# h33p/ofps

Measured on AMD Instinct MI355X. Metric: Mvectors/s, 1080p 16x16 blocks +-16 full-search SAD, higher is better.
Workload: dtype u8

## Files before the change

### ofps_amd/csrc/common.hpp

```cpp
#pragma once

#include <hip/hip_runtime.h>

#include <cstdarg>
#include <cstddef>
#include <cstdint>
#include <cstdio>
#include <cstring>
#include <string>

#include "../../include/ofps_hip.h"

namespace ofps {

int set_error(ofps_hip_ctx* ctx, int code, const char* fmt, ...);

inline int ticket_id(long number) { return (int)(number & 0x7FFFFFFF); }
inline long ticket_number(long next, int n, int id) {
    for (long k = next - 1; k >= 0 && k >= next - n; --k) if (ticket_id(k) == id) return k;
    return -1;
}

template <class Ticket, int N>
struct TicketRing {
// ... 72 lines not shown
        void* pinned = nullptr;
        int have_vectors = 0, run_detector = 0, run_estimator = 0;
        int gated = 0;
        size_t n_vectors = 0;
        IslandsTicket isl;
    };
    hipEvent_t gate_done = nullptr;
    TicketRing<Ticket, kTickets> ring;
    void release() {
        for (auto& t : ring.entry) { free_host(t.pinned); destroy(t.done); t.isl.release(); }
        for (int k = 0; k < kSlots; ++k) { destroy(uploaded[k]); destroy(slot_read[k]); }
        destroy(copy_stream); destroy(aux_stream); destroy(fork); destroy(join); destroy(gate_done);
    }
    hipError_t sync_side_streams() {
        const hipError_t e = copy_stream ? hipStreamSynchronize(copy_stream) : hipSuccess;
        return e == hipSuccess && aux_stream ? hipStreamSynchronize(aux_stream) : e;
    }
};

struct BatchStream {
    static constexpr int kTickets = 2;
    int w = 0, h = 0;
    void* last_frame = nullptr;
    struct KltPred { bool valid = false; int half = 0, w = 0, h = 0, cell = 0; uint64_t gen = 0; } klt_pred;
    struct Ticket {
        bool pending = false;
        hipEvent_t done = nullptr, uploaded = nullptr, prev_copied = nullptr;
        bool prev_copied_valid = false;
        void* pinned = nullptr; size_t pinned_cap = 0;
        int n = 0, first_has_prev = 0, run_detector = 0, run_estimator = 0;
        int filtered = 0;
        size_t n_vectors = 0;
        IslandsTicket isl;
    };
    TicketRing<Ticket, kTickets> ring;
    void release() { for (auto& t : ring.entry) { free_host(t.pinned); destroy(t.done); destroy(t.uploaded); destroy(t.prev_copied); t.isl.release(); } }
};

struct DenseStream {
    static constexpr int kSlots = 3, kTickets = 2;
    int w = 0, h = 0;
    int fw = 0, fh = 0, fmt = 0;
    long frames = 0;
    uint64_t frames_gen = 0;
    bool fb_params_valid = false; int fb_levels = 0, fb_radius = 0;
    uint64_t frame_serial = 0;
    uint64_t slot_id[kSlots] = {0, 0, 0};
    struct KltPred { bool valid = false; long pair = 0; int fw = 0, fh = 0, cell = 0; unsigned flags = 0; uint64_t gen = 0; } klt_pred;
    hipStream_t copy_stream = nullptr;
    struct Ticket {
        bool pending = false;
        hipEvent_t done = nullptr, uploaded = nullptr;
        void* pinned = nullptr; size_t pinned_cap = 0;
        int have_vectors = 0, gw = 0, gh = 0;
        size_t max_records = 0;
        int fused = 0, run_detector = 0, run_estimator = 0, dim = 0;
        size_t tail_off = 0;
        IslandsTicket isl;
    };
    TicketRing<Ticket, kTickets> ring;
    void* decode_pinned = nullptr; size_t decode_pinned_cap = 0;
    void release() {
        free_host(decode_pinned);
        for (auto& t : ring.entry) { free_host(t.pinned); destroy(t.done); destroy(t.uploaded); t.isl.release(); }
        destroy(copy_stream);
    }
    hipError_t sync_side_streams() { return copy_stream ? hipStreamSynchronize(copy_stream) : hipSuccess; }
};

}

struct ofps_hip_ctx {
    int device = 0;
    hipStream_t own_stream = nullptr;
    hipStream_t stream = nullptr;
    hipEvent_t ev_start = nullptr, ev_stop = nullptr;
    int num_cus = 0;
    int stream_cus = 0;
    int sad_mode = OFPS_HIP_SAD_EXHAUSTIVE;
    char err[512] = {0};

    struct Options {
        int sad_force_block = 0;
        int densify_no_small = 0;
        int almeida_path = 0;
        int almeida_ept = 0;
        int almeida_block = 0;
        int almeida_hier = 1;
        int almeida_fast = -1;
        int almeida_one_xcd = 1;
        int almeida_prof = 0;
        int lk_prof = 0;
        int fb_prepare_ahead = 1;
        int lk_serial = 0;
        int sad_motion_scale = 1;
        int detect_compensate = 0;
        int sad_gate = 0;
        int sad_consistency = 0;
        int sad_levels = 1;
        int sad_predictors = 0;
        int sad_median = 0;
        int sad_intra = 0;
        int sad_cut = 0;
        int sad_split = 0;
        int sad_batch_filter = 0;
        int sad_prefilter = 0;
        int detect_islands = 0;
        int klt_cell = 16, klt_score_radius = 2, klt_min_score = 1, klt_min_eig = 1, klt_max_residual = 0;
        int klt_mean_removal = 0;
        int klt_fb = 0;
        int klt_prediction = 0;
        int klt_batch_prediction = 0;
        int batch_decoder = 0, klt_levels = 4, klt_radius = 7, klt_iters = 10;
        int multi_rccl = 0;
        int test_almeida_fault = 0;
        int test_lk_fall = -1;
        int test_lk_wait_budget = 0;
        int test_lk_order = 0;
    } opt;

    ofps::PipeStream pipe;
    ofps::BatchStream batch;
    ofps::DenseStream dense;
    ofps::FarnebackState fb;
    struct IslandsLast { char* data = nullptr; size_t cap = 0; int K = 0, items = 0, dim = 0; } isl_last;
    uint32_t lk_epoch = 0;
    uint64_t lk_flags_gen = 0;

    uint32_t gran_tag_base = 0;
    uint64_t gran_zeroed_gen = 0;

    struct Scratch { void* p = nullptr; size_t cap = 0; uint64_t gen = 0; };
    static constexpr int kNumScratch = 62;
    Scratch scratch[kNumScratch];
};

namespace ofps {

enum ScratchSlot {
    S_FRAMES = 0, S_ENTRIES, S_BEST, S_FIELD, S_CELLS, S_WORK0, S_WORK1, S_WORK2, S_WORK3, S_RESULT,
    S_QUAT, S_WORK4, S_PIPE_FRAMES, S_PIPE_ENTRIES, S_PIPE_OUT, S_MASK, S_ENTRIES2, S_GRAN, S_SAD_LIST,
    S_ALM_PART, S_ALM_STATE, S_ALM_HYP, S_ALM_COUNTS, S_ALM_SEL, S_ALM_SELN, S_ALM_PROF, S_ALM_RECOVER,
    S_LK_FRAMES, S_BATCH_FRAMES, S_BATCH_ENTRIES, S_BATCH_OUT, S_BATCH_FIELD,
    S_LK_FLAGS,
    S_FB_WORK,
    S_FB_FLOW,
    S_XMAJOR,
    S_LK_MASKS,
    S_SAD_QBEST,
    S_FE_RAW,
    S_FE_RAW_PAIR,
    S_DENSE_REC,
    S_GATE_RAW,
    S_GATE_BEST,
    S_GATE_FLAGS,
    S_COMP,
    S_CONS_FWD,
    S_CONS_BWD,
    S_CONS_BWD_ENT,
    S_HIER_PYR,
    S_HIER_BEST,
    S_HIER_ENT,
    S_SAD_PREF,
    S_MED_KEEP,
    S_INTRA,
    S_ISL_WORK,
// ... 221 lines not shown
```

### ofps_amd/csrc/ctx.hip

```cpp
#include "common.hpp"

#include <cstdlib>

static thread_local char g_init_err[512] = {0};

namespace ofps {

int set_error(ofps_hip_ctx* ctx, int code, const char* fmt, ...) {
    char* dst = ctx ? ctx->err : g_init_err;
    va_list ap;
    va_start(ap, fmt);
    vsnprintf(dst, 512, fmt, ap);
    va_end(ap);
    return code;
}

int check_hip(ofps_hip_ctx* ctx, hipError_t e, const char* what) {
    if (e == hipSuccess) return OFPS_HIP_OK;
    int code = (e == hipErrorOutOfMemory) ? OFPS_HIP_ENOMEM : OFPS_HIP_EDEVICE;
    return set_error(ctx, code, "%s failed: %s", what, hipGetErrorString(e));
}

void* scratch(ofps_hip_ctx* ctx, int slot, size_t bytes) {
    auto& s = ctx->scratch[slot];
    if (bytes == 0) bytes = 16;
    if (s.cap >= bytes) return s.p;
    if (s.p) {
        if (hipStreamSynchronize(ctx->stream) != hipSuccess) {  }
        (void)hipFree(s.p);
        s.p = nullptr; s.cap = 0;
    }
    size_t cap = (bytes + 4095) & ~size_t(4095);
    hipError_t e = hipMalloc(&s.p, cap);
    if (e != hipSuccess) {
        check_hip(ctx, e, "hipMalloc(scratch)");
        s.p = nullptr;
        return nullptr;
    }
    s.cap = cap;
    s.gen += 1;
    return s.p;
}

int apply_option(ofps_hip_ctx* ctx, const char* name, const char* value, bool from_env) {
    auto& o = ctx->opt;
    const ofps_hip_ctx::Options dflt{};
    const bool unset = !value || !*value;
    const int iv = unset ? 0 : atoi(value);
    if (!strcmp(name, "OFPS_HIP_SAD_KERNEL")) {
        if (!unset && strcmp(value, "block") && strcmp(value, "strip"))
            return set_error(ctx, OFPS_HIP_EINVAL, "%s: '%s' is not block|strip", name, value);
        o.sad_force_block = !unset && !strcmp(value, "block");
    } else if (!strcmp(name, "OFPS_HIP_DENSIFY_NO_SMALL")) {
        o.densify_no_small = unset ? dflt.densify_no_small : (iv != 0);
    } else if (!strcmp(name, "OFPS_HIP_ALMEIDA_PATH")) {
        if (unset) o.almeida_path = 0;
        else if (!strcmp(value, "step")) o.almeida_path = 1;
        else if (!strcmp(value, "wg")) o.almeida_path = 2;
        else if (!strcmp(value, "cluster")) o.almeida_path = 3;
        else return set_error(ctx, OFPS_HIP_EINVAL, "%s: '%s' is not step|wg|cluster", name, value);
    } else if (!strcmp(name, "OFPS_HIP_ALMEIDA_EPT")) {
        if (!unset && iv != 1 && iv != 2 && iv != 4 && iv != 8) return set_error(ctx, OFPS_HIP_EINVAL, "%s: %d is not 1|2|4|8", name, iv);
        o.almeida_ept = unset ? 0 : iv;
    } else if (!strcmp(name, "OFPS_HIP_ALMEIDA_BLOCK")) {
        if (!unset && iv != 256 && iv != 1024) return set_error(ctx, OFPS_HIP_EINVAL, "%s: %d is not 256|1024", name, iv);
        o.almeida_block = unset ? 0 : iv;
    } else if (!strcmp(name, "OFPS_HIP_ALMEIDA_HIER")) {
        if (!unset && (iv < 0 || iv > 2)) return set_error(ctx, OFPS_HIP_EINVAL, "%s: %d is not 0|1|2", name, iv);
        o.almeida_hier = unset ? dflt.almeida_hier : iv;
    } else if (!strcmp(name, "OFPS_HIP_ALMEIDA_FAST")) {
        o.almeida_fast = unset ? -1 : (iv != 0);
    } else if (!strcmp(name, "OFPS_HIP_ALMEIDA_ONE_XCD")) {
        o.almeida_one_xcd = unset ? dflt.almeida_one_xcd : (iv != 0);
    } else if (!strcmp(name, "OFPS_HIP_ALMEIDA_PROF")) {
        o.almeida_prof = unset ? 0 : (iv != 0);
    } else if (!strcmp(name, "OFPS_HIP_LK_PROF")) {
        o.lk_prof = unset ? 0 : (iv != 0);
    } else if (!strcmp(name, "OFPS_HIP_FB_PREPARE_AHEAD")) {
        o.fb_prepare_ahead = unset ? dflt.fb_prepare_ahead : (iv != 0);
    } else if (!strcmp(name, "OFPS_HIP_LK_SERIAL")) {
        o.lk_serial = unset ? 0 : (iv != 0);
    } else if (!strcmp(name, "OFPS_HIP_SAD_MOTION_SCALE")) {
        if (!unset && iv != 1 && iv != 4) return set_error(ctx, OFPS_HIP_EINVAL, "%s: %d is not 1|4", name, iv);
        o.sad_motion_scale = unset ? dflt.sad_motion_scale : iv;
    } else if (!strcmp(name, "OFPS_HIP_DETECT_COMPENSATE")) {
        if (!unset && iv != 0 && iv != 1) return set_error(ctx, OFPS_HIP_EINVAL, "%s: %d is not 0|1", name, iv);
        o.detect_compensate = unset ? dflt.detect_compensate : iv;
    } else if (!strcmp(name, "OFPS_HIP_DETECT_ISLANDS")) {
        if (!unset && (iv < 0 || iv > kMaxIslands)) return set_error(ctx, OFPS_HIP_EINVAL, "%s: %d outside [0, %d]", name, iv, kMaxIslands);
        o.detect_islands = unset ? dflt.detect_islands : iv;
    } else if (!strcmp(name, "OFPS_HIP_SAD_GATE")) {
        if (!unset && iv < 0) return set_error(ctx, OFPS_HIP_EINVAL, "%s: %d is negative", name, iv);
        o.sad_gate = unset ? dflt.sad_gate : iv;
    } else if (!strcmp(name, "OFPS_HIP_SAD_CONSISTENCY")) {
        if (!unset && (iv < 0 || iv > kSadConsistencyMax)) return set_error(ctx, OFPS_HIP_EINVAL, "%s: %d outside [0, %d]", name, iv, kSadConsistencyMax);
        o.sad_consistency = unset ? dflt.sad_consistency : iv;
    } else if (!strcmp(name, "OFPS_HIP_SAD_MEDIAN")) {
        if (!unset && (iv < 0 || iv > kSadMedianMax)) return set_error(ctx, OFPS_HIP_EINVAL, "%s: %d outside [0, %d]", name, iv, kSadMedianMax);
        o.sad_median = unset ? dflt.sad_median : iv;
    } else if (!strcmp(name, "OFPS_HIP_SAD_INTRA")) {
        if (!unset && (iv < 0 || iv > kSadIntraMax)) return set_error(ctx, OFPS_HIP_EINVAL, "%s: %d outside [0, %d]", name, iv, kSadIntraMax);
        o.sad_intra = unset ? dflt.sad_intra : iv;
    } else if (!strcmp(name, "OFPS_HIP_SAD_CUT")) {
        if (!unset && (iv < 0 || iv > kSadCutMax)) return set_error(ctx, OFPS_HIP_EINVAL, "%s: %d outside [0, %d]", name, iv, kSadCutMax);
        o.sad_cut = unset ? dflt.sad_cut : iv;
    } else if (!strcmp(name, "OFPS_HIP_SAD_SPLIT")) {
        if (!unset && (iv < 0 || iv > kSadSplitMax)) return set_error(ctx, OFPS_HIP_EINVAL, "%s: %d outside [0, %d]", name, iv, kSadSplitMax);
        o.sad_split = unset ? dflt.sad_split : iv;
    } else if (!strcmp(name, "OFPS_HIP_SAD_LEVELS")) {
        if (!unset && (iv < 1 || iv > 3)) return set_error(ctx, OFPS_HIP_EINVAL, "%s: '%s' is not 1|2|3", name, value);
        o.sad_levels = unset ? dflt.sad_levels : iv;
    } else if (!strcmp(name, "OFPS_HIP_SAD_PREDICTORS")) {
        if (!unset && strcmp(value, "0") && strcmp(value, "1")) return set_error(ctx, OFPS_HIP_EINVAL, "%s: '%s' is not 0|1", name, value);
        o.sad_predictors = unset ? dflt.sad_predictors : iv;
    } else if (!strcmp(name, "OFPS_HIP_SAD_PREFILTER")) {
        if (!unset && (iv < 0 || iv > kSadPrefilterMax)) return set_error(ctx, OFPS_HIP_EINVAL, "%s: %d outside [0, %d]", name, iv, kSadPrefilterMax);
        o.sad_prefilter = unset ? dflt.sad_prefilter : iv;
    } else if (!strcmp(name, "OFPS_HIP_SAD_BATCH_FILTER")) {
        if (!unset && strcmp(value, "0") && strcmp(value, "1")) return set_error(ctx, OFPS_HIP_EINVAL, "%s: '%s' is not 0|1", name, value);
        o.sad_batch_filter = unset ? dflt.sad_batch_filter : iv;
    } else if (!strcmp(name, "OFPS_HIP_BATCH_DECODER")) {
        if (!unset && strcmp(value, "0") && strcmp(value, "1")) return set_error(ctx, OFPS_HIP_EINVAL, "%s: '%s' is not 0|1", name, value);
        o.batch_decoder = unset ? dflt.batch_decoder : iv;
    } else if (!strcmp(name, "OFPS_HIP_KLT_LEVELS")) {
        if (!unset && (iv < 1 || iv > kKltMaxLevels)) return set_error(ctx, OFPS_HIP_EINVAL, "%s: %d outside [1, %d]", name, iv, kKltMaxLevels);
        o.klt_levels = unset ? dflt.klt_levels : iv;
    } else if (!strcmp(name, "OFPS_HIP_KLT_RADIUS")) {
        if (!unset && (iv < 1 || iv > kKltMaxRadius)) return set_error(ctx, OFPS_HIP_EINVAL, "%s: %d outside [1, %d]", name, iv, kKltMaxRadius);
        o.klt_radius = unset ? dflt.klt_radius : iv;
    } else if (!strcmp(name, "OFPS_HIP_KLT_ITERS")) {
        if (!unset && (iv < 1 || iv > kKltMaxIters)) return set_error(ctx, OFPS_HIP_EINVAL, "%s: %d outside [1, %d]", name, iv, kKltMaxIters);
        o.klt_iters = unset ? dflt.klt_iters : iv;
    } else if (!strcmp(name, "OFPS_HIP_KLT_CELL")) {
        if (!unset && iv != 8 && iv != 16 && iv != 32) return set_error(ctx, OFPS_HIP_EINVAL, "%s: %d is not 8|16|32", name, iv);
        o.klt_cell = unset ? dflt.klt_cell : iv;
    } else if (!strcmp(name, "OFPS_HIP_KLT_SCORE_RADIUS")) {
        if (!unset && (iv < 1 || iv > kKltMaxScoreRadius)) return set_error(ctx, OFPS_HIP_EINVAL, "%s: %d outside [1, %d]", name, iv, kKltMaxScoreRadius);
        o.klt_score_radius = unset ? dflt.klt_score_radius : iv;
    } else if (!strcmp(name, "OFPS_HIP_KLT_MIN_SCORE")) {
        if (!unset && iv < 1) return set_error(ctx, OFPS_HIP_EINVAL, "%s: %d is below 1", name, iv);
        o.klt_min_score = unset ? dflt.klt_min_score : iv;
    } else if (!strcmp(name, "OFPS_HIP_KLT_MIN_EIG")) {
        if (!unset && (iv < 1 || iv > kKltMaxMinEig)) return set_error(ctx, OFPS_HIP_EINVAL, "%s: %d outside [1, %d]", name, iv, kKltMaxMinEig);
        o.klt_min_eig = unset ? dflt.klt_min_eig : iv;
    } else if (!strcmp(name, "OFPS_HIP_KLT_MAX_RESIDUAL")) {
        if (!unset && (iv < 0 || iv > kKltMaxResidual)) return set_error(ctx, OFPS_HIP_EINVAL, "%s: %d outside [0, %d]", name, iv, kKltMaxResidual);
        o.klt_max_residual = unset ? dflt.klt_max_residual : iv;
    } else if (!strcmp(name, "OFPS_HIP_KLT_MEAN_REMOVAL")) {
        if (!unset && strcmp(value, "0") && strcmp(value, "1")) return set_error(ctx, OFPS_HIP_EINVAL, "%s: '%s' is not 0|1", name, value);
        o.klt_mean_removal = unset ? dflt.klt_mean_removal : iv;
    } else if (!strcmp(name, "OFPS_HIP_KLT_FB")) {
        if (!unset && (strspn(value, "0123456789") != strlen(value) || strlen(value) > 4 || iv > kKltMaxFb)) return set_error(ctx, OFPS_HIP_EINVAL, "%s: '%s' outside [0, %d]", name, value, kKltMaxFb);
        o.klt_fb = unset ? dflt.klt_fb : iv;
    } else if (!strcmp(name, "OFPS_HIP_KLT_PREDICTION")) {
        if (!unset && strcmp(value, "0") && strcmp(value, "1")) return set_error(ctx, OFPS_HIP_EINVAL, "%s: '%s' is not 0|1", name, value);
        o.klt_prediction = unset ? dflt.klt_prediction : iv;
    } else if (!strcmp(name, "OFPS_HIP_KLT_BATCH_PREDICTION")) {
        if (!unset && strcmp(value, "0") && strcmp(value, "1")) return set_error(ctx, OFPS_HIP_EINVAL, "%s: '%s' is not 0|1", name, value);
        o.klt_batch_prediction = unset ? dflt.klt_batch_prediction : iv;
    } else if (!strcmp(name, "OFPS_HIP_MULTI_RCCL")) {
        o.multi_rccl = unset ? 0 : (iv != 0);
    } else if (!strcmp(name, "OFPS_HIP_ALMEIDA_TEST_FAULT") || !strcmp(name, "OFPS_HIP_LK_TEST_FALL") ||
               !strcmp(name, "OFPS_HIP_LK_TEST_WAIT_BUDGET") || !strcmp(name, "OFPS_HIP_LK_TEST_ORDER")) {
#ifdef OFPS_HIP_TEST_HOOKS
        if (from_env) return OFPS_HIP_OK;
        if (!strcmp(name, "OFPS_HIP_ALMEIDA_TEST_FAULT")) o.test_almeida_fault = unset ? 0 : iv;
        else if (!strcmp(name, "OFPS_HIP_LK_TEST_WAIT_BUDGET")) o.test_lk_wait_budget = unset || iv < 0 ? 0 : iv;
        else if (!strcmp(name, "OFPS_HIP_LK_TEST_ORDER")) o.test_lk_order = unset || iv < 0 || iv > 2 ? 0 : iv;
        else o.test_lk_fall = unset ? -1 : iv;
#else
        if (from_env) return OFPS_HIP_OK;
        return set_error(ctx, OFPS_HIP_EUNSUPPORTED, "%s is a test hook: this library was built without OFPS_HIP_TEST_HOOKS", name);
#endif
    } else {
        return set_error(ctx, OFPS_HIP_EINVAL, "unknown option '%s'", name);
    }
    return OFPS_HIP_OK;
}

static const char* const kOptionNames[] = {
    "OFPS_HIP_SAD_KERNEL", "OFPS_HIP_DENSIFY_NO_SMALL", "OFPS_HIP_ALMEIDA_PATH", "OFPS_HIP_ALMEIDA_EPT", "OFPS_HIP_ALMEIDA_BLOCK",
    "OFPS_HIP_ALMEIDA_HIER", "OFPS_HIP_ALMEIDA_FAST", "OFPS_HIP_ALMEIDA_ONE_XCD", "OFPS_HIP_ALMEIDA_PROF", "OFPS_HIP_LK_PROF", "OFPS_HIP_LK_SERIAL", "OFPS_HIP_FB_PREPARE_AHEAD", "OFPS_HIP_MULTI_RCCL",
    "OFPS_HIP_SAD_MOTION_SCALE", "OFPS_HIP_DETECT_COMPENSATE", "OFPS_HIP_SAD_GATE", "OFPS_HIP_SAD_CONSISTENCY", "OFPS_HIP_SAD_LEVELS",
    "OFPS_HIP_SAD_PREDICTORS", "OFPS_HIP_SAD_PREFILTER", "OFPS_HIP_SAD_MEDIAN", "OFPS_HIP_SAD_BATCH_FILTER",
    "OFPS_HIP_SAD_INTRA", "OFPS_HIP_SAD_CUT", "OFPS_HIP_DETECT_ISLANDS", "OFPS_HIP_SAD_SPLIT",
    "OFPS_HIP_KLT_CELL", "OFPS_HIP_KLT_SCORE_RADIUS", "OFPS_HIP_KLT_MIN_SCORE", "OFPS_HIP_KLT_MIN_EIG", "OFPS_HIP_KLT_MAX_RESIDUAL",
    "OFPS_HIP_BATCH_DECODER", "OFPS_HIP_KLT_LEVELS", "OFPS_HIP_KLT_RADIUS", "OFPS_HIP_KLT_ITERS", "OFPS_HIP_KLT_MEAN_REMOVAL",
    "OFPS_HIP_KLT_FB", "OFPS_HIP_KLT_PREDICTION", "OFPS_HIP_KLT_BATCH_PREDICTION"};

}

extern "C" {

int ofps_hip_api_version(void) { return OFPS_HIP_API_VERSION; }

int ofps_hip_device_count(void) {
    int n = 0;
    if (hipGetDeviceCount(&n) != hipSuccess) return 0;
    return n;
}

static int stream_cu_count(ofps_hip_ctx* ctx, hipStream_t s);

int ofps_hip_init(int device, ofps_hip_ctx** out) {
    if (!out) return ofps::set_error(nullptr, OFPS_HIP_EINVAL, "ofps_hip_init: out is NULL");
    *out = nullptr;
    int n = 0;
    hipError_t e = hipGetDeviceCount(&n);
    if (e != hipSuccess || n <= 0)
        return ofps::set_error(nullptr, OFPS_HIP_EDEVICE,
                               "ofps_hip_init: no HIP device (%s); this backend has no CPU fallback",
                               e == hipSuccess ? "count == 0" : hipGetErrorString(e));
    if (device < 0 || device >= n)
        return ofps::set_error(nullptr, OFPS_HIP_EINVAL, "ofps_hip_init: device %d out of range [0,%d)", device, n);
    hipDeviceProp_t prop;
    e = hipGetDeviceProperties(&prop, device);
    if (e != hipSuccess) return ofps::check_hip(nullptr, e, "hipGetDeviceProperties");
    if (strncmp(prop.gcnArchName, "gfx950", 6) != 0)
        return ofps::set_error(nullptr, OFPS_HIP_EUNSUPPORTED,
                               "ofps_hip_init: device %d is %s; this library ships gfx950 code only", device,
                               prop.gcnArchName);
    auto* ctx = new ofps_hip_ctx();
    ctx->device = device;
    ctx->num_cus = prop.multiProcessorCount;
    if ((e = hipSetDevice(device)) != hipSuccess ||
        (e = hipStreamCreateWithFlags(&ctx->own_stream, hipStreamNonBlocking)) != hipSuccess ||
        (e = hipEventCreate(&ctx->ev_start)) != hipSuccess || (e = hipEventCreate(&ctx->ev_stop)) != hipSuccess) {
        int rc = ofps::check_hip(nullptr, e, "context setup");
        delete ctx;
        return rc;
    }
    ctx->stream = ctx->own_stream;
    ctx->stream_cus = stream_cu_count(ctx, ctx->stream);
    for (const char* name : ofps::kOptionNames)
        if (const char* v = getenv(name)) {
            if (ofps::apply_option(ctx, name, v, true) != OFPS_HIP_OK) {
                fprintf(stderr, "[ofps_hip] warning: ignoring environment variable %s=%s (%s)\n", name, v, ctx->err);
                ctx->err[0] = '\0';
            }
        }
    ofps::cluster_gate_context_created(device);
    *out = ctx;
    return OFPS_HIP_OK;
}

int ofps_hip_set_option(ofps_hip_ctx* ctx, const char* name, const char* value) {
    if (!ctx) return OFPS_HIP_EINVAL;
    OFPS_REQUIRE(ctx, name, "set_option: null name");
    return ofps::apply_option(ctx, name, value, false);
}

int ofps_hip_has_test_hooks(void) {
#ifdef OFPS_HIP_TEST_HOOKS
    return 1;
#else
    return 0;
#endif
}

int ofps_hip_almeida_recoveries(ofps_hip_ctx* ctx, uint64_t* count) {
    if (!ctx || !count) return OFPS_HIP_EINVAL;
    *count = 0;
    const void* d = ctx->scratch[ofps::S_ALM_RECOVER].p;
    if (!d) return OFPS_HIP_OK;
// ... 125 lines not shown
```

### ofps_amd/csrc/sad.hip

```cpp
#include "common.hpp"

#include <cstdlib>
#include <utility>

namespace {

constexpr int kWavesPerWG = 4;

constexpr int pick_stride(int min_s, int k, int ng) {
    for (int s = min_s; s < min_s + 64; ++s)
        if ((k * s) % 32 == ng % 32) return s;
    return min_s | 1;
}

template <int B, int R, int K>
struct SadCfg {
    static_assert(B % 4 == 0 && R % 4 == 0, "tile origin must stay dword aligned");
    static_assert(B * B * 255 <= 65535, "packed u16 SAD accumulators would overflow");
    static constexpr int NCAND = 2 * R + 1;
    static constexpr int NG = (NCAND + 3) / 4;
    static constexpr int NC = (NCAND + K - 1) / K;
    static constexpr int T = NG * NC;
    static constexpr int PASSES = (T + 63) / 64;
    static constexpr int BW = B / 4;
// ... 790 lines not shown
    }
    const int dy0i = blk_on ? (int)((pbest >> 8) & 0xFF) : R, dx0i = blk_on ? (int)(pbest & 0xFF) : R;
    auto key64 = [&](uint32_t sad, int dyi, int dxi) {
        const int dy = dyi - R, dx = dxi - R;
        return ((unsigned long long)((sad << 16) | (uint32_t)(dx * dx + dy * dy)) << 32) | (unsigned long long)(uint32_t)((dyi << 8) | dxi);
    };
    uint32_t U = pde_two_rows(tile, curl, b, dy0i, dx0i, g);
#pragma unroll
    for (int m = 1; m < C::NG; m <<= 1) U += __shfl_xor(U, m, 64);
    if (g == 0) bestk[b] = blk_on ? key64(U, dy0i, dx0i) : ~0ull;
    int nlist = 0;
    {
        int uj[4];
#pragma unroll
        for (int j = 0; j < 4; ++j) uj[j] = colv[j] ? (int)U : -1;
        const unsigned long long below = (1ull << lane) - 1ull;
        typedef unsigned short us2 __attribute__((ext_vector_type(2)));
        const uint32_t u1 = min(U + 1u, 0xFFFFu) * 0x10001u;
        auto any_le = [&](uint32_t v) {
            const us2 m = __builtin_elementwise_min(__builtin_bit_cast(us2, v), __builtin_bit_cast(us2, u1));
            return __builtin_bit_cast(uint32_t, m) ^ u1;
        };
#pragma unroll
        for (int i = 0; i < C::NCAND; ++i) {
            const int dy = -R + i;
            if (y0 + dy >= 0 && y0 + dy + B <= p.H) {
                const uint32_t lo = (uint32_t)acc[i], hi = (uint32_t)(acc[i] >> 32);
                if (!__ballot((any_le(lo) | any_le(hi)) != 0u)) continue;
                const int s4[4] = {(int)(lo & 0xFFFFu), (int)(lo >> 16), (int)(hi & 0xFFFFu), (int)(hi >> 16)};
#pragma unroll
                for (int j = 0; j < 4; ++j) {
                    const bool hit = s4[j] <= uj[j];
                    const unsigned long long mask = __ballot(hit);
                    if (mask) {
                        const int pos = nlist + __popcll(mask & below);
                        if (hit && pos < P::CAP) list[pos] = ((uint32_t)b << 16) | ((uint32_t)i << 8) | (uint32_t)(4 * g + j);
                        nlist += __popcll(mask);
                    }
                }
            }
        }
#pragma unroll
        for (int i = 0; i < C::KE; ++i) {
            const int dyi = g * C::KE + i, dy = dyi - R;
            const bool hit = xok && dy <= R && y0 + dy >= 0 && y0 + dy + B <= p.H && eacc[i] <= U;
            const unsigned long long mask = __ballot(hit);
            if (mask) {
                const int pos = nlist + __popcll(mask & below);
                if (hit && pos < P::CAP) list[pos] = ((uint32_t)b << 16) | ((uint32_t)dyi << 8) | (uint32_t)(2 * R);
                nlist += __popcll(mask);
            }
        }
    }
    __builtin_amdgcn_fence(__ATOMIC_RELEASE, "wavefront");
    __builtin_amdgcn_wave_barrier();
    __builtin_amdgcn_fence(__ATOMIC_ACQUIRE, "wavefront");
    const int n = nlist;
    if (n > P::CAP) {
        if (lane == 0) {
            const uint32_t pos = atomicAdd(&strip_list[0], 1u);
            strip_list[1 + pos] = (uint32_t)strip;
        }
        return;
    }
    constexpr int PER_STEP = 2 * (64 / C::NG);
    for (int base = 0; base < n; base += PER_STEP) {
        const int idx0 = base + lane / C::NG, idx1 = idx0 + 64 / C::NG;
        const uint32_t e0 = list[min(idx0, n - 1)], e1 = list[min(idx1, n - 1)];
        const int bb0 = (int)(e0 >> 16), dyi0 = (int)((e0 >> 8) & 0xFF), dxi0 = (int)(e0 & 0xFF);
        const int bb1 = (int)(e1 >> 16), dyi1 = (int)((e1 >> 8) & 0xFF), dxi1 = (int)(e1 & 0xFF);
        uint32_t s0 = pde_two_rows(tile, curl, bb0, dyi0, dxi0, g);
        uint32_t s1 = pde_two_rows(tile, curl, bb1, dyi1, dxi1, g);
#pragma unroll
        for (int m = 1; m < C::NG; m <<= 1) { s0 += __shfl_xor(s0, m, 64); s1 += __shfl_xor(s1, m, 64); }
        if (g == 0 && idx0 < n) atomicMin(&bestk[bb0], key64(s0, dyi0, dxi0));
        if (g == 0 && idx1 < n) atomicMin(&bestk[bb1], key64(s1, dyi1, dxi1));
    }
    __builtin_amdgcn_fence(__ATOMIC_RELEASE, "wavefront");
    __builtin_amdgcn_wave_barrier();
    __builtin_amdgcn_fence(__ATOMIC_ACQUIRE, "wavefront");
    if (blk_on && g == 0) write_block_result(p, pair, bx, by, B, R, bestk[b]);
}

__global__ __launch_bounds__(64) void sad_generic_kernel(const SadParams p, int B, int R) {
    const int pair = blockIdx.z, by = blockIdx.y, bx = blockIdx.x;
    const uint8_t* __restrict__ prev = p.prev_base + (size_t)pair * p.prev_pitch;
    const uint8_t* __restrict__ cur = p.cur_base + (size_t)pair * p.cur_pitch;
    const int x0 = bx * B, y0 = by * B, n = 2 * R + 1;
    unsigned long long best = ~0ull;
    for (int cand = threadIdx.x; cand < n * n; cand += 64) {
        const int dy = cand / n - R, dx = cand % n - R;
        if (x0 + dx < 0 || x0 + dx + B > p.W || y0 + dy < 0 || y0 + dy + B > p.H) continue;
        uint32_t sad = 0;
        for (int y = 0; y < B; ++y) {
            const uint8_t* cr = cur + (size_t)(y0 + y) * p.stride + x0;
            const uint8_t* pr = prev + (size_t)(y0 + dy + y) * p.stride + x0 + dx;
            for (int x = 0; x < B; ++x) {
                const int d = (int)cr[x] - (int)pr[x];
                sad += (uint32_t)(d < 0 ? -d : d);
            }
        }
        const unsigned long long key = ((unsigned long long)sad << 32) | ((unsigned long long)(dx * dx + dy * dy) << 16) |
                                       (unsigned long long)(((dy + R) << 8) | (dx + R));
        best = key < best ? key : best;
    }
#pragma unroll
    for (int m = 32; m >= 1; m >>= 1) {
        const unsigned long long o = shfl_xor_u64(best, m);
        best = o < best ? o : best;
    }
    if (threadIdx.x == 0) {
        const int sad = (int)(best >> 32);
        const int dy = (int)((best >> 8) & 0xFF) - R, dx = (int)(best & 0xFF) - R;
        const size_t k = ((size_t)pair * p.nby + by) * p.nbx + bx;
        float4 e;
        e.x = (float)(x0 + B / 2 + dx) * p.nx;
        e.y = (float)(y0 + B / 2 + dy) * p.ny;
        e.z = ((float)dx / 1.0f) * (-p.nx);
        e.w = ((float)dy / 1.0f) * (-p.ny);
        p.out_entries[k] = e;
        if (p.out_best) {
            p.out_best[3 * k + 0] = dx;
            p.out_best[3 * k + 1] = dy;
            p.out_best[3 * k + 2] = sad;
        }
    }
}

template <int B, int R, int K>
void launch_qsad(const SadParams& p, int pairs, hipStream_t s) {
    dim3 grid((p.nbx + kWavesPerWG - 1) / kWavesPerWG, p.nby, pairs);
    hipLaunchKernelGGL((sad_qsad_kernel<B, R, K>), grid, dim3(256), 0, s, p);
}

inline void strip_div_magic(SadParams& q, int strips_per_row) {
    q.div_spp = div_magic48((unsigned)strips_per_row * (unsigned)q.nby);
    q.div_spr = div_magic48((unsigned)strips_per_row);
}

template <int B, int R>
void launch_strip(const SadParams& p, int pairs, hipStream_t s) {
    using C = StripCfg<B, R>;
    const int strips_per_row = (p.nbx + C::NB - 1) / C::NB;
    const int total = strips_per_row * p.nby * pairs;
    const int nwg = ((total + kStripWaves - 1) / kStripWaves + 7) / 8 * 8;
    SadParams q = p;
    strip_div_magic(q, strips_per_row);
    hipLaunchKernelGGL((sad_strip_kernel<B, R>), dim3(nwg), dim3(64 * kStripWaves), 0, s, q, strips_per_row, total);
}

int launch_pde_16_16(ofps_hip_ctx* ctx, const SadParams& p, int pairs, hipStream_t s) {
    using C = StripCfg<16, 16>;
    const int strips_per_row = (p.nbx + C::NB - 1) / C::NB;
    const int total = strips_per_row * p.nby * pairs;
    auto* strip_list = static_cast<uint32_t*>(ofps::scratch(ctx, ofps::S_SAD_LIST, (size_t)(total + 1) * sizeof(uint32_t)));
    if (!strip_list) return OFPS_HIP_ENOMEM;
    OFPS_HIP_TRY(ctx, hipMemsetAsync(strip_list, 0, sizeof(uint32_t), s));
    const int nwg = ((total + kStripWaves - 1) / kStripWaves + 7) / 8 * 8;
    hipLaunchKernelGGL(sad_pde_kernel, dim3(nwg), dim3(64 * kStripWaves), 0, s, p, strips_per_row, total, strip_list);
    const int nwg_ind = nwg < 8 * ctx->num_cus ? nwg : 8 * ctx->num_cus;
    SadParams q = p;
    strip_div_magic(q, strips_per_row);
    hipLaunchKernelGGL((sad_strip_list_kernel<16, 16>), dim3(nwg_ind), dim3(64 * kStripWaves), 0, s, q, strips_per_row,
                       (const uint32_t*)strip_list);
    return OFPS_HIP_OK;
}

}

extern "C" {

size_t ofps_hip_sad_block_count(int W, int H, int block) {
    if (W <= 0 || H <= 0 || block <= 0) return 0;
    return (size_t)(W / block) * (size_t)(H / block);
}

}

namespace {
int sad_check_args(ofps_hip_ctx* ctx, const ofps::SadFrames& f, int block, int range) {
    OFPS_REQUIRE(ctx, f.W > 0 && f.H > 0 && f.stride >= f.W, "sad_flow: bad geometry W=%d H=%d stride=%d", f.W, f.H, f.stride);
    OFPS_REQUIRE(ctx, f.stride % 4 == 0 && ((uintptr_t)f.prev_base % 4) == 0 && ((uintptr_t)f.cur_base % 4) == 0 &&
                          f.prev_pitch % 4 == 0 && f.cur_pitch % 4 == 0,
                 "sad_flow: rows must be 4-byte aligned (stride=%d)", f.stride);
    OFPS_REQUIRE(ctx, block >= 1 && block <= 64 && range >= 0 && range <= 64,
                 "sad_flow: block=%d range=%d outside [1,64]/[0,64]", block, range);
    return OFPS_HIP_OK;
}

SadParams sad_params(const ofps::SadFrames& f, int block, void* d_out_entries, void* d_out_best) {
    SadParams p{};
    p.prev_base = f.prev_base; p.cur_base = f.cur_base;
    p.prev_pitch = f.prev_pitch; p.cur_pitch = f.cur_pitch;
    p.W = f.W; p.H = f.H; p.stride = f.stride;
    p.nbx = f.W / block; p.nby = f.H / block;
    p.nx = 1.0f / (float)f.W; p.ny = 1.0f / (float)f.H;
    p.out_entries = static_cast<float4*>(d_out_entries);
    p.out_best = static_cast<int*>(d_out_best);
    return p;
}

int sad_launch(ofps_hip_ctx* ctx, const ofps::SadFrames& f, int pairs, int block, int range, void* d_out_entries, void* d_out_best) {
    const SadParams p = sad_params(f, block, d_out_entries, d_out_best);
    hipStream_t s = ctx->stream;
    const int key = block * 1000 + range;
    const bool force_block = ctx->opt.sad_force_block != 0;
    const bool strip_ok = !force_block && f.stride % 16 == 0 && ((uintptr_t)f.prev_base % 16) == 0 &&
                          ((uintptr_t)f.cur_base % 16) == 0 && f.prev_pitch % 16 == 0 && f.cur_pitch % 16 == 0 &&
                          (long long)p.nbx * p.nby * pairs < (1ll << 28) && (long long)p.nbx * p.nby < (1ll << 20);
    switch (key) {
        case 16016:
            if (strip_ok && ctx->sad_mode == OFPS_HIP_SAD_PRUNED) {
                const int rc = launch_pde_16_16(ctx, p, pairs, s);
                if (rc != OFPS_HIP_OK) return rc;
            } else if (strip_ok) launch_strip<16, 16>(p, pairs, s);
            else launch_qsad<16, 16, 5>(p, pairs, s);
            break;
        case 16008:
            if (strip_ok) launch_strip<16, 8>(p, pairs, s); else launch_qsad<16, 8, 3>(p, pairs, s);
            break;
        case 16032:
            if (strip_ok) launch_strip<16, 32>(p, pairs, s); else launch_qsad<16, 32, 5>(p, pairs, s);
            break;
        case 8032:
            if (strip_ok) launch_strip<8, 32>(p, pairs, s); else launch_qsad<8, 32, 5>(p, pairs, s);
            break;
        case 8016:
            if (strip_ok) launch_strip<8, 16>(p, pairs, s); else launch_qsad<8, 16, 5>(p, pairs, s);
            break;
        case 8008:
            if (strip_ok) launch_strip<8, 8>(p, pairs, s); else launch_qsad<8, 8, 3>(p, pairs, s);
            break;
#define OFPS_STRIP_CASE(BB, RR)                                         \
        case BB * 1000 + RR:                                            \
            if (strip_ok) { launch_strip<BB, RR>(p, pairs, s); break; } \
            [[fallthrough]];
        OFPS_STRIP_CASE(16, 12) OFPS_STRIP_CASE(16, 20) OFPS_STRIP_CASE(16, 24) OFPS_STRIP_CASE(16, 28)
// ... 128 lines not shown
```

Baseline: 525.6.

## Replace two-kernel PDE SAD with single-pass row-chunk pruning kernel

Adds a single kernel for the 16x16 +-16 full search. It computes a partial SAD over a row subset, takes an upper bound from the best candidate's full SAD, and then finishes only the dy chunks that still hold a live candidate, falling back to all chunks once enough rows survive. This replaces the previous PDE kernel plus indirect strip-list kernel, removing the second launch and its list traffic. The cost is more register pressure, wavefront-scope LDS atomics for the per-column minima, and a new tunable density threshold option.

```diff
diff --git a/ofps_amd/csrc/common.hpp b/ofps_amd/csrc/common.hpp
--- a/ofps_amd/csrc/common.hpp
+++ b/ofps_amd/csrc/common.hpp
@@ -178,6 +178,7 @@
 
     struct Options {
         int sad_force_block = 0;
+        int sad_pde_dense = 34;
         int densify_no_small = 0;
         int almeida_path = 0;
         int almeida_ept = 0;
diff --git a/ofps_amd/csrc/ctx.hip b/ofps_amd/csrc/ctx.hip
--- a/ofps_amd/csrc/ctx.hip
+++ b/ofps_amd/csrc/ctx.hip
@@ -51,6 +51,9 @@
         if (!unset && strcmp(value, "block") && strcmp(value, "strip"))
             return set_error(ctx, OFPS_HIP_EINVAL, "%s: '%s' is not block|strip", name, value);
         o.sad_force_block = !unset && !strcmp(value, "block");
+    } else if (!strcmp(name, "OFPS_HIP_SAD_PDE_DENSE")) {
+        if (!unset && (strspn(value, "0123456789") != strlen(value) || strlen(value) > 2)) return set_error(ctx, OFPS_HIP_EINVAL, "%s: '%s' outside [0, 99]", name, value);
+        o.sad_pde_dense = unset ? dflt.sad_pde_dense : iv;
     } else if (!strcmp(name, "OFPS_HIP_DENSIFY_NO_SMALL")) {
         o.densify_no_small = unset ? dflt.densify_no_small : (iv != 0);
     } else if (!strcmp(name, "OFPS_HIP_ALMEIDA_PATH")) {
@@ -179,7 +182,7 @@
 }
 
 static const char* const kOptionNames[] = {
-    "OFPS_HIP_SAD_KERNEL", "OFPS_HIP_DENSIFY_NO_SMALL", "OFPS_HIP_ALMEIDA_PATH", "OFPS_HIP_ALMEIDA_EPT", "OFPS_HIP_ALMEIDA_BLOCK",
+    "OFPS_HIP_SAD_KERNEL", "OFPS_HIP_SAD_PDE_DENSE", "OFPS_HIP_DENSIFY_NO_SMALL", "OFPS_HIP_ALMEIDA_PATH", "OFPS_HIP_ALMEIDA_EPT", "OFPS_HIP_ALMEIDA_BLOCK",
     "OFPS_HIP_ALMEIDA_HIER", "OFPS_HIP_ALMEIDA_FAST", "OFPS_HIP_ALMEIDA_ONE_XCD", "OFPS_HIP_ALMEIDA_PROF", "OFPS_HIP_LK_PROF", "OFPS_HIP_LK_SERIAL", "OFPS_HIP_FB_PREPARE_AHEAD", "OFPS_HIP_MULTI_RCCL",
     "OFPS_HIP_SAD_MOTION_SCALE", "OFPS_HIP_DETECT_COMPENSATE", "OFPS_HIP_SAD_GATE", "OFPS_HIP_SAD_CONSISTENCY", "OFPS_HIP_SAD_LEVELS",
     "OFPS_HIP_SAD_PREDICTORS", "OFPS_HIP_SAD_PREFILTER", "OFPS_HIP_SAD_MEDIAN", "OFPS_HIP_SAD_BATCH_FILTER",
diff --git a/ofps_amd/csrc/sad.hip b/ofps_amd/csrc/sad.hip
--- a/ofps_amd/csrc/sad.hip
+++ b/ofps_amd/csrc/sad.hip
@@ -896,6 +896,338 @@
     if (blk_on && g == 0) write_block_result(p, pair, bx, by, B, R, bestk[b]);
 }
 
+#ifndef OFPS_SAD_PDE
+#define OFPS_SAD_PDE 2
+#endif
+constexpr int kSadPde = OFPS_SAD_PDE;
+
+struct PdeRowsCfg {
+    static constexpr int B = 16, R = 16;
+    using C = StripCfg<B, R>;
+    static constexpr int TILE_DW = C::TILE_H * C::SW;
+    static constexpr int CUR_DW = PdeCfg::CUR_DW;
+    static constexpr int OFF_CUR = TILE_DW, OFF_MIN = OFF_CUR + CUR_DW;
+    static constexpr int WAVE_DW = OFF_MIN + 4 * 64;
+    static_assert(C::COMPACT_KEY && C::SPLIT == 1 && C::NP == C::NCAND, "written for the +-16 geometry");
+    static_assert((C::NG - 1) * C::KE2 + B + C::KE2 - 2 < C::TILE_H, "the dx = +R chunks must stay inside the window");
+};
+
+__device__ __forceinline__ void pde_fold(unsigned long long a, uint32_t low, uint32_t hmask, uint32_t* amin) {
+    const uint32_t lo = (uint32_t)a, hi = (uint32_t)(a >> 32);
+    const uint32_t k[4] = {(lo << 16) | low, (lo & hmask) | low, (hi << 16) | low, (hi & hmask) | low};
+#pragma unroll
+    for (int j = 0; j < 4; ++j) __hip_atomic_fetch_min(amin + 64 * j, k[j], __ATOMIC_RELAXED, __HIP_MEMORY_SCOPE_WAVEFRONT);
+}
+
+#ifndef OFPS_SAD_PDE_CH
+#define OFPS_SAD_PDE_CH 3
+#endif
+constexpr int PDE_CH = OFPS_SAD_PDE_CH;
+template <int K>
+__device__ __forceinline__ void pde_chunk(unsigned long long take, int ilo, int ihi, unsigned long long (&acc)[PdeRowsCfg::C::NP],
+                                          const uint32_t (&c)[PdeRowsCfg::B][PdeRowsCfg::C::BW], const uint32_t* lds, uint32_t tile_off,
+                                          uint32_t hmask, uint32_t* amin) {
+    using C = PdeRowsCfg::C;
+    constexpr int B = PdeRowsCfg::B, R = PdeRowsCfg::R;
+    constexpr int I0 = K * PDE_CH, N = I0 + PDE_CH <= C::NCAND ? PDE_CH : C::NCAND - I0;
+    constexpr int ROWS = N + B - 2;
+    constexpr int GR = (255 - C::BW) / C::SW + 1;
+    if ((take >> K) & 1ull) {
+        uint32_t base = tile_off + (I0 + 1) * C::SW;
+        asm volatile("" : "+v"(base));
+        auto load = [&](int r, unsigned long long (&w)[C::BW]) {
+            if (r > 0 && r % GR == 0) {
+                base += GR * C::SW;
+                asm volatile("" : "+v"(base));
+            }
+#pragma unroll
+            for (int q = 0; q < C::BW; ++q) w[q] = reinterpret_cast<const U64A4*>(lds + base + (r % GR) * C::SW + q)->v;
+        };
+        unsigned long long nxt[C::BW];
+        load(0, nxt);
+#pragma unroll
+        for (int r = 0; r < ROWS; ++r) {
+            unsigned long long win[C::BW];
+#pragma unroll
+            for (int q = 0; q < C::BW; ++q) win[q] = nxt[q];
+            if (r + 1 < ROWS) load(r + 1, nxt);
+#pragma unroll
+            for (int ii = 0; ii < N; ++ii) {
+                const int y = r + 1 - ii;
+                if (y >= 1 && y < B && y % PdeCfg::STEP != 0) {
+#pragma unroll
+                    for (int q = 0; q < C::BW; ++q) acc[I0 + ii] = __builtin_amdgcn_qsad_pk_u16_u8(win[q], c[y][q], acc[I0 + ii]);
+                }
+            }
+            asm volatile("" : : : "memory");
+        }
+#pragma unroll
+        for (int ii = 0; ii < N; ++ii) {
+            const int i = I0 + ii, dy = i - R;
+            pde_fold(acc[i], (i >= ilo && i <= ihi) ? (uint32_t)((dy * dy) << 6 | i) : 0xFFFFFFFFu, hmask, amin);
+        }
+    }
+}
+template <int... K>
+__device__ __forceinline__ void pde_chunks(unsigned long long take, int ilo, int ihi, unsigned long long (&acc)[PdeRowsCfg::C::NP],
+                                           const uint32_t (&c)[PdeRowsCfg::B][PdeRowsCfg::C::BW], const uint32_t* lds, uint32_t tile_off,
+                                           uint32_t hmask, uint32_t* amin, std::integer_sequence<int, K...>) {
+    (pde_chunk<K>(take, ilo, ihi, acc, c, lds, tile_off, hmask, amin), ...);
+}
+
+__global__ __launch_bounds__(64 * kStripWaves, 3) void sad_pde_rows_kernel(const SadParams p, int strips_per_row, int total_strips, int dense_t,
+                                                                           uint32_t* __restrict__ unpruned) {
+    using P = PdeRowsCfg;
+    using C = P::C;
+    constexpr int B = P::B, R = P::R;
+    __shared__ __attribute__((aligned(16))) uint32_t lds[kStripWaves * P::WAVE_DW];
+
+    const int wave = __builtin_amdgcn_readfirstlane(threadIdx.x >> 6);
+    const int lane = threadIdx.x & 63;
+    const int per_xcd = gridDim.x / 8;
+    const int lwg = (int)(blockIdx.x % 8) * per_xcd + (int)(blockIdx.x / 8);
+    const int strip = lwg * kStripWaves + wave;
+    if (strip >= total_strips) return;
+    const int strips_per_pair = strips_per_row * p.nby;
+    const int pair = (int)div48((unsigned)strip, p.div_spp);
+    const int rem = strip - pair * strips_per_pair;
+    const int by = (int)div48((unsigned)rem, p.div_spr);
+    const int bx0 = (rem - by * strips_per_row) * C::NB;
+    const uint8_t* __restrict__ prev = p.prev_base + (size_t)pair * p.prev_pitch;
+    const uint8_t* __restrict__ cur = p.cur_base + (size_t)pair * p.cur_pitch;
+    uint32_t* tile = lds + wave * P::WAVE_DW;
+    uint32_t* curl = tile + P::OFF_CUR;
+    uint32_t* amin = tile + P::OFF_MIN + lane;
+
+    const int b = lane / C::NG, g = lane % C::NG;
+    const int bx = bx0 + b;
+    const bool blk_on = bx < p.nbx;
+    const int y0 = by * B;
+
+    {
+        constexpr int LR = 64 / C::TILE_WG;
+        constexpr int STEPS = (C::TILE_H + LR - 1) / LR;
+        const int tx0 = bx0 * B - R, ty0 = y0 - R;
+        const int sr = lane / C::TILE_WG, sc = lane - sr * C::TILE_WG;
+        const int gx = tx0 + C::GRAN * sc;
+        const bool lane_on = sr < LR && gx >= 0 && gx < p.W;
+        const uint8_t* src = prev + (ptrdiff_t)(ty0 + sr) * p.stride + gx;
+        uint32_t* dst = tile + sr * C::SW + C::GDW * sc;
+        static_assert(C::GRAN == 16, "16-byte granules");
+#pragma unroll
+        for (int it = 0; it < STEPS; ++it) {
+            const int row = sr + it * LR;
+            const bool row_in_tile = (it + 1) * LR <= C::TILE_H || row < C::TILE_H;
+            if (lane_on && row_in_tile && (unsigned)(ty0 + row) < (unsigned)p.H)
+                *reinterpret_cast<uint4*>(dst + it * LR * C::SW) = *reinterpret_cast<const uint4*>(src + (ptrdiff_t)(it * LR) * p.stride);
+        }
+#pragma unroll
+        for (int k = 0; k < 2; ++k) {
+            const int idx = lane + 64 * k, row = idx / C::NB, blk = idx % C::NB;
+            const int bxc = min(bx0 + blk, p.nbx - 1);
+            *reinterpret_cast<uint4*>(curl + row * (C::NB * C::BW) + blk * C::BW) =
+                *reinterpret_cast<const uint4*>(cur + (size_t)(y0 + row) * p.stride + bxc * B);
+        }
+#pragma unroll
+        for (int j = 0; j < 4; ++j) amin[64 * j] = 0xFFFFFFFFu;
+    }
+    __builtin_amdgcn_fence(__ATOMIC_RELEASE, "wavefront");
+    __builtin_amdgcn_wave_barrier();
+    __builtin_amdgcn_fence(__ATOMIC_ACQUIRE, "wavefront");
+
+    const int ilo = __builtin_amdgcn_readfirstlane(R - y0 > 0 ? R - y0 : 0);
+    const int ihi = __builtin_amdgcn_readfirstlane(p.H - B - y0 < R ? R + p.H - B - y0 : 2 * R);
+    const uint32_t lane_off = (uint32_t)(wave * P::WAVE_DW + b * C::BW + g);
+    const uint32_t* cblk = curl + b * C::BW;
+
+    unsigned long long acc[C::NP];
+#pragma unroll
+    for (int ii = 0; ii < C::NP; ++ii) acc[ii] = 0;
+    {
+        uint32_t c4[PdeCfg::PR][C::BW];
+#pragma unroll
+        for (int r = 0; r < PdeCfg::PR; ++r)
+#pragma unroll
+            for (int q = 0; q < C::BW; ++q) c4[r][q] = cblk[(PdeCfg::STEP * r) * (C::NB * C::BW) + q];
+        pde_rows(acc, c4, lds, lane_off, std::make_integer_sequence<int, C::NCAND + B - 1>{});
+    }
+#pragma unroll
+    for (int ii = 0; ii < C::NP; ++ii) asm volatile("" : "+v"(acc[ii]));
+
+    const int dx0 = -R + 4 * g;
+    uint32_t colk[4];
+#pragma unroll
+    for (int j = 0; j < 4; ++j) {
+        const int x = bx * B + dx0 + j;
+        colk[j] = (blk_on && x >= 0 && x + B <= p.W) ? (uint32_t)((dx0 + j) * (dx0 + j)) << C::KSHIFT : 0xFFFFFFFFu;
+    }
+    uint32_t U;
+    {
+        uint32_t pkey = 0xFFFFFFFFu;
+#pragma unroll
+        for (int i = 0; i < C::NCAND; ++i) {
+            if (i >= ilo && i <= ihi) {
+                const int dy = -R + i;
+                const uint32_t lo = (uint32_t)acc[i], hi = (uint32_t)(acc[i] >> 32);
+                const uint32_t k0 = (lo << 16) | colk[0], k1 = (lo & 0xFFFF0000u) | colk[1];
+                const uint32_t k2 = (hi << 16) | colk[2], k3 = (hi & 0xFFFF0000u) | colk[3];
+                pkey = min(pkey, __builtin_elementwise_add_sat(min(min(k0, k1), min(k2, k3)), (uint32_t)((dy * dy) << 6 | i)));
+            }
+        }
+        unsigned long long pbest = ~0ull;
+        if (pkey != 0xFFFFFFFFu) {
+            const int bi = (int)(pkey & 63u), dy = -R + bi;
+            const uint32_t d2 = (pkey & 0xFFFFu) >> C::KSHIFT;
+            const int dxsq = (int)d2 - dy * dy;
+            int dx = dx0;
+#pragma unroll
+            for (int j = 1; j < 4; ++j) dx = ((dx0 + j) * (dx0 + j) == dxsq) ? dx0 + j : dx;
+            pbest = ((unsigned long long)((pkey & 0xFFFF0000u) | d2) << 32) | (unsigned long long)(uint32_t)(((dy + R) << 8) | (dx + R));
+        }
+#pragma unroll
+        for (int m = 1; m < C::NG; m <<= 1) {
+            const unsigned long long o = shfl_xor_u64(pbest, m);
+            pbest = o < pbest ? o : pbest;
+        }
+        const bool have = blk_on && pbest != ~0ull;
+        const int dy0i = have ? (int)((pbest >> 8) & 0xFF) : R, dx0i = have ? (int)(pbest & 0xFF) : R;
+        U = pde_two_rows(tile, curl, b, dy0i, dx0i, g);
+#pragma unroll
+        for (int m = 1; m < C::NG; m <<= 1) U += __shfl_xor(U, m, 64);
+        U = have ? U : 0xFFFFFFFFu;
+    }
+    unsigned long long live = 0;
+    {
+        typedef unsigned short us2 __attribute__((ext_vector_type(2)));
+        const uint32_t u1 = U == 0xFFFFFFFFu ? 0u : (U + 1u) * 0x10001u;
+        auto any_le = [&](uint32_t v) {
+            const us2 m = __builtin_elementwise_min(__builtin_bit_cast(us2, v), __builtin_bit_cast(us2, u1));
+            return __builtin_bit_cast(uint32_t, m) ^ u1;
+        };
+#pragma unroll
+        for (int i = 0; i < C::NCAND; ++i) {
+            if (i >= ilo && i <= ihi) {
+                const uint32_t lo = (uint32_t)acc[i], hi = (uint32_t)(acc[i] >> 32);
+                if (__ballot((any_le(lo) | any_le(hi)) != 0u)) live |= 1ull << i;
+            }
+        }
+    }
+    uint32_t hmask = 0xFFFF0000u;
+    asm volatile("" : "+v"(hmask));
+    {
+        constexpr int NCH = (C::NCAND + PDE_CH - 1) / PDE_CH;
+        const bool dense = __popcll(live) >= dense_t;
+        unsigned long long take = 0, in_frame = 0;
+#pragma unroll
+        for (int k = 0; k < NCH; ++k) {
+            const unsigned long long rows = ((1ull << PDE_CH) - 1ull) << (k * PDE_CH);
+            in_frame |= (k * PDE_CH <= ihi && k * PDE_CH + PDE_CH - 1 >= ilo) ? 1ull << k : 0ull;
+            take |= (live & rows) != 0ull ? 1ull << k : 0ull;
+        }
+        take = dense ? in_frame : take;
+        if (take == in_frame && lane == 0) atomicAdd(unpruned, 1u);
+        uint32_t c[B][C::BW];
+#pragma unroll
+        for (int y = 0; y < B; ++y)
+#pragma unroll
+            for (int q = 0; q < C::BW; ++q) c[y][q] = y % PdeCfg::STEP != 0 ? cblk[y * (C::NB * C::BW) + q] : 0u;
+        pde_chunks(take, ilo, ihi, acc, c, lds, lane_off, hmask, amin, std::make_integer_sequence<int, NCH>{});
+    }
+    uint32_t bkey = 0xFFFFFFFFu;
+#pragma unroll
+    for (int j = 0; j < 4; ++j) {
+        const uint32_t kc = __hip_atomic_load(amin + 64 * j, __ATOMIC_RELAXED, __HIP_MEMORY_SCOPE_WAVEFRONT);
+        uint32_t lk = (kc & 0xFFFF0000u) | ((kc & 0xFFFFu) + colk[j]);
+        lk = (colk[j] == 0xFFFFFFFFu || kc == 0xFFFFFFFFu) ? 0xFFFFFFFFu : lk;
+        bkey = min(bkey, lk);
+    }
+    unsigned long long best = ~0ull;
+    if (bkey != 0xFFFFFFFFu) {
+        const uint32_t d2 = (bkey & 0xFFFFu) >> C::KSHIFT;
+        const int dy = -R + (int)(bkey & 63u);
+        const int dxsq = (int)d2 - dy * dy;
+        int dx = dx0;
+#pragma unroll
+        for (int j = 1; j < 4; ++j) dx = ((dx0 + j) * (dx0 + j) == dxsq) ? dx0 + j : dx;
+        best = ((unsigned long long)((bkey & 0xFFFF0000u) | d2) << 32) | (unsigned long long)(uint32_t)(((dy + R) << 8) | (dx + R));
+    }
+    {
+        asm volatile("" : : : "memory");
+        uint32_t c[B][C::BW];
+#pragma unroll
+        for (int y = 0; y < B; ++y)
+#pragma unroll
+            for (int q = 0; q < C::BW; ++q) c[y][q] = cblk[y * (C::NB * C::BW) + q];
+        uint32_t eacc[C::KE2];
+#pragma unroll
+        for (int i = 0; i < C::KE2; ++i) eacc[i] = 0;
+        const uint32_t* ecol = tile + b * C::BW + C::EDGE_COL;
+        const int erow0 = g * C::KE2;
+        uint32_t nxt[C::BW];
+#pragma unroll
+        for (int q = 0; q < C::BW; ++q) nxt[q] = ecol[erow0 * C::SW + q];
+#pragma unroll
+        for (int rr = 0; rr < B + C::KE2 - 1; ++rr) {
+            uint32_t ref[C::BW];
+#pragma unroll
+            for (int q = 0; q < C::BW; ++q) ref[q] = nxt[q];
+            if (rr + 1 < B + C::KE2 - 1) {
+#pragma unroll
+                for (int q = 0; q < C::BW; ++q) nxt[q] = ecol[(erow0 + rr + 1) * C::SW + q];
+            }
+#pragma unroll
+            for (int i = 0; i < C::KE2; ++i) {
+                const int y = rr - i;
+                if (y >= 0 && y < B) {
+#pragma unroll
+                    for (int q = 0; q < C::BW; ++q) eacc[i] = __builtin_amdgcn_sad_u8(ref[q], c[y][q], eacc[i]);
+                }
+            }
+            asm volatile("" : "+v"(eacc[0]) : : "memory");
+        }
+#pragma unroll
+        for (int i = 1; i < C::KE2; ++i) asm volatile("" : "+v"(eacc[i]));
+        static_assert(C::NG * C::ERL == B, "the lanes of a block share the rows of dy = +R evenly");
+        uint32_t elast = 0;
+#pragma unroll
+        for (int r = 0; r < C::ERL; ++r) {
+            const int y = g * C::ERL + r;
+#pragma unroll
+            for (int q = 0; q < C::BW; ++q) elast = __builtin_amdgcn_sad_u8(ecol[(2 * R + y) * C::SW + q], cblk[y * (C::NB * C::BW) + q], elast);
+        }
+#pragma unroll
+        for (int m = 1; m < C::NG; m <<= 1) elast += (uint32_t)__shfl_xor((int)elast, m, 64);
+
+        const bool xok = blk_on && bx * B + R + B <= p.W;
+        const int chi = ihi < 2 * R - 1 ? ihi : 2 * R - 1;
+        uint32_t ek = 0xFFFFFFFFu;
+        int ei = 0;
+#pragma unroll
+        for (int i = 0; i < C::KE2; ++i) {
+            const int idx = g * C::KE2 + i, dy = idx - R;
+            const bool v = (unsigned)(idx - ilo) <= (unsigned)(chi - ilo);
+            const uint32_t k = v ? ((eacc[i] << 16) | (uint32_t)(R * R + dy * dy)) : 0xFFFFFFFFu;
+            const bool lt = k < ek;
+            ek = lt ? k : ek;
+            ei = lt ? idx : ei;
+        }
+        if (ihi == 2 * R) {
+            const uint32_t k = (elast << 16) | (uint32_t)(2 * R * R);
+            const bool lt = k < ek;
+            ek = lt ? k : ek;
+            ei = lt ? 2 * R : ei;
+        }
+        const unsigned long long k64 = ((unsigned long long)ek << 32) | (unsigned long long)(uint32_t)((ei << 8) | (2 * R));
+        best = (xok && ek != 0xFFFFFFFFu && k64 < best) ? k64 : best;
+    }
+#pragma unroll
+    for (int m = 1; m < C::NG; m <<= 1) {
+        const unsigned long long o = shfl_xor_u64(best, m);
+        best = o < best ? o : best;
+    }
+    if (blk_on && g == 0) write_block_result(p, pair, bx, by, B, R, best);
+}
+
 __global__ __launch_bounds__(64) void sad_generic_kernel(const SadParams p, int B, int R) {
     const int pair = blockIdx.z, by = blockIdx.y, bx = blockIdx.x;
     const uint8_t* __restrict__ prev = p.prev_base + (size_t)pair * p.prev_pitch;
@@ -967,6 +1299,16 @@
     using C = StripCfg<16, 16>;
     const int strips_per_row = (p.nbx + C::NB - 1) / C::NB;
     const int total = strips_per_row * p.nby * pairs;
+    if constexpr (kSadPde != 1) {
+        auto* unpruned = static_cast<uint32_t*>(ofps::scratch(ctx, ofps::S_SAD_LIST, sizeof(uint32_t)));
+        if (!unpruned) return OFPS_HIP_ENOMEM;
+        OFPS_HIP_TRY(ctx, hipMemsetAsync(unpruned, 0, sizeof(uint32_t), s));
+        const int nwg = ((total + kStripWaves - 1) / kStripWaves + 7) / 8 * 8;
+        SadParams q = p;
+        strip_div_magic(q, strips_per_row);
+        hipLaunchKernelGGL(sad_pde_rows_kernel, dim3(nwg), dim3(64 * kStripWaves), 0, s, q, strips_per_row, total, ctx->opt.sad_pde_dense, unpruned);
+        return OFPS_HIP_OK;
+    }
     auto* strip_list = static_cast<uint32_t*>(ofps::scratch(ctx, ofps::S_SAD_LIST, (size_t)(total + 1) * sizeof(uint32_t)));
     if (!strip_list) return OFPS_HIP_ENOMEM;
     OFPS_HIP_TRY(ctx, hipMemsetAsync(strip_list, 0, sizeof(uint32_t), s));
```

Result: no change. 526.2, median of 6 (+0.1%).
